# Geronimorz/MCMC-in-Tonga

Hardware: AMD Instinct MI355X
Metric: MCMC proposals/sec (likelihood evals/sec) at 381 rays x N cells (higher is better)
Workload: dtype f64

## Files before the change

### mcmc-in-tonga_amd/csrc/chain_kernels.hip

```cpp
#pragma clang fp contract(off)

#include <hip/hip_runtime.h>

#include <algorithm>
#include <atomic>
#include <climits>
#include <cstddef>
#include <cstdlib>

#include "chain_dev.h"
#include "chain_diag.h"
#include "chain_resident.h"
#include "chain_search.h"
#include "chain_shared.h"
#include "chain_tiles.h"
#include "chain_variant.h"
#include "exact_sum.h"
#include "internal.h"
#include "ray_sum.h"
#include "wave_ops.h"

namespace tdstar {

namespace {
// ... 284 lines not shown
    if constexpr (SMALL && !RLDS) {
        float *a = reinterpret_cast<float *>(lds + L.tlo), *b = reinterpret_cast<float *>(lds + L.thi);
        double *m = reinterpret_cast<double *>(lds + L.tmaxd);
        int *ts = reinterpret_cast<int *>(lds + L.tstart), *tr = reinterpret_cast<int *>(lds + L.tray);
        {
            constexpr int U = 4;
            CopySeg<float, U, NTH> c0{a, d.tile_lo, 3 * NT}, c1{b, d.tile_hi, 3 * NT};
            CopySeg<double, U, NTH> c2{m, d.tile_maxd, NT};
            CopySeg<int, U, NTH> c7{ts, d.tile_start, NT + 1}, c8{tr, d.tile_ray, NT};
            for (int b0 = tid; b0 < 3 * NT; b0 += U * NTH) {
                c0.load(b0); c1.load(b0); c2.load(b0); c7.load(b0); c8.load(b0);
                c0.store(b0); c1.store(b0); c2.store(b0); c7.store(b0); c8.store(b0);
            }
        }
        v.tlo = a; v.thi = b; v.tmaxd = m; v.tstart = ts; v.tray = tr;
        v.thit = reinterpret_cast<int *>(lds + L.thit);
        v.ctm = reinterpret_cast<double *>(lds + L.ctm);
        v.ctm_cap = kCtmLds;
        __syncthreads();
    }
    if constexpr (RLDS) {
        float *a = reinterpret_cast<float *>(lds + L.tlo), *b = reinterpret_cast<float *>(lds + L.thi);
        double *m = reinterpret_cast<double *>(lds + L.tmaxd);
        int *ts = reinterpret_cast<int *>(lds + L.tstart), *ro = reinterpret_cast<int *>(lds + L.rayoff);
        double *p = reinterpret_cast<double *>(lds + L.ptS), *pf = reinterpret_cast<double *>(lds + L.prefix);
        double *t = reinterpret_cast<double *>(lds + L.tS), *sg = reinterpret_cast<double *>(lds + L.sig);
        int *rf = reinterpret_cast<int *>(lds + L.rflag), *od = reinterpret_cast<int *>(lds + L.ord);
        int *tr = reinterpret_cast<int *>(lds + L.tray);
        v.tray = tr;
        {
            constexpr int U = 4;
            CopySeg<float, U, NTH> c0{a, d.tile_lo, 3 * NT}, c1{b, d.tile_hi, 3 * NT};
            CopySeg<double, U, NTH> c2{m, d.tile_maxd, NT}, c3{p, d.ptS, n}, c4{pf, d.prefix, n}, c5{t, d.tS, n},
                c6{sg, d.sig, n};
            CopySeg<int, U, NTH> c7{ts, d.tile_start, NT + 1}, c8{tr, d.tile_ray, NT}, c9{ro, d.ray_off, n + 1},
                c10{od, d.order, d.st->ncells};
            const int most = max(max(3 * NT, NT + 1), max(n + 1, c10.n));
            for (int b0 = tid; b0 < most; b0 += U * NTH) {
                c0.load(b0); c1.load(b0); c2.load(b0); c3.load(b0); c4.load(b0); c5.load(b0);
                c6.load(b0); c7.load(b0); c8.load(b0); c9.load(b0); c10.load(b0);
                c0.store(b0); c1.store(b0); c2.store(b0); c3.store(b0); c4.store(b0); c5.store(b0);
                c6.store(b0); c7.store(b0); c8.store(b0); c9.store(b0); c10.store(b0);
            }
        }
        for (int i = tid; i < n; i += NTH) rf[i] = 0;
        v.tlo = a; v.thi = b; v.tmaxd = m; v.tstart = ts; v.ray_off = ro; v.ptS = p; v.prefix = pf; v.tS = t;
        v.sig = sg; v.rflag = rf; v.ord = od;
        v.cptS = reinterpret_cast<double *>(lds + L.cptS);
        v.cprefix = reinterpret_cast<double *>(lds + L.cprefix);
        v.term = reinterpret_cast<double *>(lds + L.term);
        v.cterm = reinterpret_cast<double *>(lds + L.cterm);
        v.thit = reinterpret_cast<int *>(lds + L.thit);
        v.ctm = reinterpret_cast<double *>(lds + L.ctm);
        v.ctm_cap = NT + 1;
        v.rhit = reinterpret_cast<int *>(lds + L.rhit);
        v.rhit_cap = n;
        __syncthreads();
    }
    const long long t_mirror = prof_on ? clock64() : 0;
    {
        double part = 0.0;
        for (int r = tid; r < n; r += NTH) {
            const double df = v.ptS[r] - v.tS[r];
            const double sg = v.sig[r];
            const double t = ((df * df) * 1.0) / (sg * sg);
            v.term[r] = t;
            part = part + t;
        }
        if constexpr (!RLDS) {
            part = wave_sum_f64(part);
            if (lane == 0) sh.wpart[wv] = part;
        }
    }
    if (tid == 0) {
        const ChainScalars &s0 = *d.st;
        sh.iter = s0.iter;
        sh.evaluations = 0;
        sh.bytes = 0;
        sh.cur = 0;
        sh.defer = 0;
        if (!RLDS) sh.dsum = sh.dabs = 0.0;
        sh.grid_fallbacks32 = 0;
        sh.e_done = sh.b_done = 0;
        geo_fill(sh.geo, d);
        for (int a = 0; a < 5; ++a) sh.proposed[a] = sh.accepted[a] = 0;
        sh.phi = s0.phi;
        sh.ncells = s0.ncells;
        for (int k = 0; k < 3; ++k) sh.lnN[k] = d.logN[max(s0.ncells - 1 + k, 0)];
        sh.nslots = s0.nslots;
        sh.nfree = s0.nfree;
        sh.next_stamp = s0.next_stamp;
        sh.g_op = 0;
        sh.grid_ovf = *d.grid_overflow;
        sh.rT = P.temperature;
        sh.rinv2t = P.inv_2t;
        sh.srv_quit = 0;
        sh.rK = 0;
        for (int k = 0; k < kProfSlots; ++k) sh.prof[k] = 0;
        sh.t_last = clock64();
        sh.dseg.nseg = 0;
    }
    __syncthreads();
    const long long t_init = prof_on ? clock64() : 0;
    unsigned long long *smask = reinterpret_cast<unsigned long long *>(lds + L.smask);
    unsigned long long *cmask = reinterpret_cast<unsigned long long *>(lds + L.cmask);
    const int NS = d.nsuper;
    float *slo = reinterpret_cast<float *>(lds + L.slo), *shi = reinterpret_cast<float *>(lds + L.shi);
    float *smax = reinterpret_cast<float *>(lds + L.smax);
    int *shit = reinterpret_cast<int *>(lds + L.shit);
    const bool super_on = !SMALL && L.super_lds;
    if constexpr (WALK) {
        if constexpr (SMALL) __syncthreads();
        delta_marks(v.term, v.prefix, nullptr, n, smask, wv, delta_words(n), kWv, lane);
        for (int w = tid; w < delta_words(n); w += NTH) cmask[w] = 0ull;
    }
    if constexpr (!SMALL) {
        if (super_on) {
            for (int i = tid; i < 3 * NS; i += NTH) {
                slo[i] = d.super_lo[i];
                shi[i] = d.super_hi[i];
            }
            for (int S = tid; S < NS; S += NTH) {
                double m = 0.0;
                for (int t = S * kTilePts; t < min(NT, (S + 1) * kTilePts); ++t) m = fmax(m, d.tile_maxd[t]);
                smax[S] = f32_up(m);
            }
            if (tid == 0) sh.n_super[0] = sh.n_super[1] = 0;
        }
        __syncthreads();
    }

    if (wv == 0) {
        if (sa.pre) {
            if (lane < iters) draws[lane] = sa.pre[(long long)bchain * sa.pre_stride + lane];
        } else if (!nscript) {
            draws[lane] = tdchain::draw_iteration(d.seed, d.chain, (uint64_t)(sh.iter + lane));
        }
        wave_sync_lds();
        if (mb) {
            if (lane == 0) {
                sh.srv_seq = mb_load(&mb->done);
                sh.srv_quit = 0;
                sh.srv_busy_c = 0;
            }
            wave_sync_lds();
            server_wait(mb, d, v, sh, lane);
        }
        if (rbx) {
            if (lane == 0) sh.rseq = mb_load(&rbx->slot[bchain].done);
            wave_sync_lds();
            round_wait(rbx, bchain, sh, lane, false, sh.phi);
        }
        if (lane == 0 && iters > 0 && !((mb || rbx) && sh.srv_quit)) {
            if (nscript) {
                sh.step_cur = mb ? sh.srv_step[sh.srv_k++] : sa.step[0];
                script_proposal(sh.ps[0], sh.step_cur, sh.nfree, sh.nslots, d.free_slots,
                                [&](int pos) { return v.ord[pos]; });
            }
            else
                make_proposal(sh.ps[0], P, draws[0], sh.ncells, sh.nfree, sh.nslots, d.free_slots, d.cx, d.cy, d.cz,
                              d.czeta, [&](int pos) { return v.ord[pos]; });
            if (sh.ps[0].p.active) sh.proposed[sh.ps[0].p.action] += 1;
            sh.n_tiles = sh.n_changed = sh.n_orphans = sh.n_rays = 0;
            sh.pts_seen = sh.ray_pts = 0;
            sh.k0 = n;
            sh.gs.accept = 0;
// ... 15 lines not shown
            sh.prof[73] += t_init - t_mirror;
            sh.prof[74] += t_now - t_init;
        }
    }
    double phi_r = sh.phi;
    double inv2t_r = sh.rinv2t;
    long long round_end = rbx ? sh.rK : xch ? (long long)rxp->K : LLONG_MAX;
    int cur_r = 0;
    bool pend_r = false;
    bool pend_sup = false;
    int last_action = 0, last_accept = 0;
    long long it_done = 0;
    long long rec_next = LLONG_MAX;
    if constexpr (REC && !ROUNDS)
        if (d.rec.every > 0 && !rbx) rec_next = d.rec.first;
    if constexpr (REC && ROUNDS)
        if (tid == 0) sh.mbox[0] = sh.mbox[1] = -1;
    if (tid == 0) {
        sh.ex_upto = n;
        sh.phi_lo = sh.phi_hi = phi_r;
        if constexpr (!RLDS) {
            double T = 0.0;
            for (int w = 0; w < kWv; ++w) T = T + sh.wpart[w];
            sh.tsum = T;
            sh.terr = kSumSlack * (double)(n + 1) * fabs(T);
        }
    }
    __syncthreads();
    for (long long it = 0; it < iters && !((mb || rbx || xch) && sh.srv_quit); ++it) {
        if (prof_on && tid == 0) sh.t_iter = clock64();
        int sup_n = 0, sup_S = 0, sup_par = 0;
        bool sup_all = false;
        unsigned long long sup_mk = 0ull;
        if constexpr (!SMALL) {
            if (pend_sup) {
                sup_par = (int)((it - 1) & 1);
                const int nsh = sh.n_super[sup_par];
                sup_all = nsh > kListLds;
                sup_n = sup_all ? NS : nsh;
                if ((tid >> 4) < sup_n) {
                    sup_S = sup_all ? (tid >> 4) : shit[sup_par * kListLds + (tid >> 4)];
                    const int t = sup_S * kTilePts + (tid & 15);
                    sup_mk = t < NT ? (unsigned long long)__double_as_longlong(d.tile_maxd[t]) : 0ull;
                }
            }
        }
        if constexpr (WALK) {
            if (pend_r) delta_commit<SMALL ? 1 : 16>(v.prefix, v.cprefix, n, sh.dseg, tid, NTH);
            pend_r = false;
        }
        if constexpr (!SMALL) {
            if (pend_sup) {
                if ((tid >> 4) < sup_n) {
                    const unsigned long long mk = row_max_u64(sup_mk);
                    if ((tid & 15) == 15) smax[sup_S] = f32_up(__longlong_as_double((long long)mk));
                }
                for (int i = (tid >> 4) + NTH / kTilePts; i < sup_n; i += NTH / kTilePts) {
                    const int S = sup_all ? i : shit[sup_par * kListLds + i], t = S * kTilePts + (tid & 15);
                    unsigned long long mk = t < NT ? (unsigned long long)__double_as_longlong(d.tile_maxd[t]) : 0ull;
                    mk = row_max_u64(mk);
                    if ((tid & 15) == 15) smax[S] = f32_up(__longlong_as_double((long long)mk));
                }
                __syncthreads();
                SKEW(1);
                pend_sup = false;
            }
        }
        bool acc_r = false;
        const PState &cur = sh.ps[sh.cur];
        const Proposal p = cur.p;
        const int action = p.action;
        const int ncells = sh.ncells;
        const int slot_k = cur.slot_k;
        const bool eval = cur.eval != 0;
        const double kx = cur.kx, ky = cur.ky, kz = cur.kz;
        const int new_slot = cur.new_slot;
        const double zeta_killed = cur.zeta_killed;
        double czeta = 0.0, zetanew_death = 0.0;
        STAMP(0);
        bool pre_on = false;
        bool nobar = false;
        int pre_q = 0, pre_ray = 0, pre_s = 0;
        double pre_bd = 0.0, pre_x = 0.0, pre_y = 0.0, pre_z = 0.0;
        const bool sroad = !SCRIPT && cur.barren != 0 && p.active && p.valid && P.debug_prior != 1 &&
                           (action == tdchain::kChange || action == tdchain::kDeath);
        if (p.active) {
            const bool kill_q = SCRIPT && mb && action == tdchain::kDeath && sh.step_cur.decision == kDecideLater;
            const bool query = (!nscript && (action == tdchain::kBirth || action == tdchain::kDeath)) || kill_q;
            nobar = kNoBarB && action != tdchain::kBirth && p.valid && P.debug_prior != 1 && !sroad;
            if (eval && !sroad) {
                const bool q0 = action != tdchain::kBirth;
                const bool q1 = action == tdchain::kBirth || action == tdchain::kMove;
                const TileQuery tq0 = tile_query(kx, ky, kz), tq1 = tile_query(p.x, p.y, p.z);
                const int nthr = query ? NTH - 64 : NTH;
                constexpr int TU = SMALL ? 3 : 8;
                if (super_on) {
                    const int par = (int)(it & 1);
                    int *hl = shit + par * kListLds;
                    if (tid < nthr)
                        for (int S0 = tid; S0 < NS; S0 += 4 * nthr) {
                            bool hit[4];
#pragma unroll
                            for (int u = 0; u < 4; ++u) {
                                const int S = min(S0 + u * nthr, NS - 1);
                                const float thr = smax[S] * (1.0f + 0x1p-20f);
                                const bool h0 = tile_may_hit(slo, shi, NS, S, tq0, thr);
                                const bool h1 = tile_may_hit(slo, shi, NS, S, tq1, thr);
                                hit[u] = S0 + u * nthr < NS && ((q0 && h0) || (q1 && h1));
                            }
#pragma unroll
                            for (int u = 0; u < 4; ++u)
                                if (hit[u]) {
                                    const int k = atomicAdd(&sh.n_super[par], 1);
                                    if (k < kListLds) hl[k] = S0 + u * nthr;
                                }
                        }
                    __syncthreads();
                    SKEW(2);
                    const int nsh = sh.n_super[par];
                    const bool all = nsh > kListLds;
                    const int nitems = all ? NS * kTilePts : nsh * kTilePts;
                    if (tid < nthr)
                        for (int i0 = tid; i0 < nitems; i0 += 4 * nthr) {
                            bool hit[4];
                            int4 rec[4];
#pragma unroll
                            for (int u = 0; u < 4; ++u) {
                                const int i = min(i0 + u * nthr, nitems - 1);
                                const int tu = (all ? (i >> 4) : hl[i >> 4]) * kTilePts + (i & 15);
                                const int t = min(tu, NT - 1);
                                const float thr = tile_thr(v.tmaxd[t]);
                                const bool h0 = tile_may_hit(v.tlo, v.thi, NT, t, tq0, thr);
                                const bool h1 = tile_may_hit(v.tlo, v.thi, NT, t, tq1, thr);
                                rec[u] = int4{t, v.tstart[t], v.tray[t], 0};
                                hit[u] = i0 + u * nthr < nitems && tu < NT && ((q0 && h0) || (q1 && h1));
                            }
#pragma unroll
                            for (int u = 0; u < 4; ++u)
                                if (hit[u]) {
                                    const int k = atomicAdd(&sh.n_tiles, 1);
                                    v.thit[k] = rec[u].x;
                                    if (k < v.hrec_cap) v.hrec[k] = rec[u];
                                }
                        }
                } else if (SMALL) {
                    const TileQuery2 tr0 = tile_query2(kx, ky, kz), tr1 = tile_query2(p.x, p.y, p.z);
                    if (tid < nthr) {
                        int npre = 0;
                        int pt[kPre] = {0, 0, 0, 0};
                        for (int b0 = wv * 64; b0 < NT; b0 += TU * nthr) {
                            const int t0 = b0 + lane;
                            bool hit[TU];
                            if constexpr (TD_TILE2) {
                                TileBox bx[TU];
#pragma unroll
                                for (int u = 0; u < TU; ++u)
                                    bx[u] = tile_box(v.tlo, v.thi, v.tmaxd, NT, min(t0 + u * nthr, NT - 1));
                                const int au = __builtin_amdgcn_readfirstlane(action);
                                const bool s0 = au != tdchain::kBirth, s1 = au == tdchain::kBirth || au == tdchain::kMove;
#pragma unroll
                                for (int u = 0; u < TU; ++u) hit[u] = false;
                                if (s0) {
#pragma unroll
                                    for (int u = 0; u < TU; ++u) hit[u] = tile_may_hit2(bx[u], tr0);
                                }
                                if (s1) {
#pragma unroll
                                    for (int u = 0; u < TU; ++u) hit[u] = hit[u] || tile_may_hit2(bx[u], tr1);
// ... 10 lines not shown
                                    hit[u] = t0 + u * nthr < NT && ((q0 && h0) || (q1 && h1));
                                }
                            }
#pragma unroll
                            for (int u = 0; u < TU; ++u) {
                                const unsigned long long m = __ballot(hit[u]);
                                if (m == 0ull) continue;
                                const int first = __builtin_ctzll(m), cnt = __popcll(m);
                                const int rank = __popcll(m & ((1ull << lane) - 1ull));
                                int base = 0;
                                if (lane == first) base = atomicAdd(&sh.n_tiles, cnt);
                                base = __builtin_amdgcn_readlane(base, first);
                                if (hit[u]) {
                                    const int t = t0 + u * nthr, slot = npre + rank;
                                    v.thit[base + rank] = slot < kPre ? (t | INT_MIN) : t;
                                }
                                for (unsigned long long mm = m; mm && npre < kPre; mm &= mm - 1ull) {
                                    const int t = b0 + __builtin_ctzll(mm) + u * nthr;
#pragma unroll
                                    for (int k = 0; k < kPre; ++k) pt[k] = k == npre ? t : pt[k];
                                    ++npre;
                                }
                            }
                        }
                        BPROBE(0);
                        if (npre > 0) {
                            if (lane < kTilePts * npre) {
                                const int g = lane / kTilePts;
                                const int t = g == 0 ? pt[0] : g == 1 ? pt[1] : g == 2 ? pt[2] : pt[3];
                                const int sc = v.tstart[t];
                                if (lane % kTilePts < (sc & 31)) {
                                    const int q = (sc >> 5) + lane % kTilePts;
                                    pre_on = true;
                                    pre_q = q;
                                    pre_ray = v.tray[t];
                                    pre_s = d.best_s[q];
                                    pre_bd = d.best_d[q];
                                    pre_x = d.px[q];
                                    pre_y = d.py[q];
                                    pre_z = d.pz[q];
                                }
                            }
                        }
                    }
                } else if (tid < nthr)
                    for (int t0 = tid; t0 < NT; t0 += TU * nthr) {
                        bool hit[TU];
#pragma unroll
                        for (int u = 0; u < TU; ++u) {
                            const int t = min(t0 + u * nthr, NT - 1);
                            const float thr = tile_thr(v.tmaxd[t]);
                            const bool h0 = tile_may_hit(v.tlo, v.thi, NT, t, tq0, thr);
                            const bool h1 = tile_may_hit(v.tlo, v.thi, NT, t, tq1, thr);
                            hit[u] = t0 + u * nthr < NT && ((q0 && h0) || (q1 && h1));
                        }
#pragma unroll
                        for (int u = 0; u < TU; ++u)
                            if (hit[u]) {
                                const int k = atomicAdd(&sh.n_tiles, 1), t = t0 + u * nthr;
                                v.thit[k] = t;
                                if (!SMALL && k < v.hrec_cap) v.hrec[k] = int4{t, v.tstart[t], v.tray[t], 0};
                            }
                    }
            }
            BPROBE(1);
            if (nobar && !(query && wv == kWv - 1)) {
                __builtin_amdgcn_fence(__ATOMIC_RELEASE, "workgroup");
                if (lane == 0) atomicAdd(&sh.b_done, 1);
                SKEW(3);
            }
            if (RLDS && action == tdchain::kDeath && nscript) {
                const int sthr = query ? NTH - 64 : NTH;
                if constexpr (RLDS) {
                    if (tid < sthr)
                        for (int j = (int)p.index + 1 + tid; j < ncells; j += sthr) d.order_tmp[j] = v.ord[j];
                }
            }
            if (query && wv == kWv - 1) {
                const bool birth = action == tdchain::kBirth;
                if (nobar && lane == 0) atomicAdd(&sh.b_done, 1);
                const Nearest r = wave_nearest(d, v, sh, lane, birth ? p.x : kx, birth ? p.y : ky, birth ? p.z : kz,
                                               birth ? -1 : slot_k, -1, 0.0, 0.0, 0.0, 0.0);
                if (lane == 0) sh.q_zeta = r.z;
            }
        }
        if (!nobar && !(sroad && action == tdchain::kChange)) {
            __syncthreads();
            SKEW(4);
            if (p.active && action == tdchain::kBirth) czeta = sh.q_zeta;
            if (p.active && action == tdchain::kDeath) zetanew_death = sh.q_zeta;
        }
        BPROBE(2);
        Proposal pp = p;
        if (p.active && action == tdchain::kBirth && !nscript) tdchain::birth_zeta(P, pp, czeta);
        STAMP(1);
        const bool can_spec = !nscript && it + 1 < iters && ((it + 1) & 63) != 0;
        if (pp.active && pp.valid) {
            const bool fwd = P.debug_prior != 1;
            int no = 0;
            if (fwd && !sroad) {
                if (!nscript && tid == NTH - 64)
                    sh.ap = tdchain::alpha_parts(P, pp, czeta, zeta_killed,
                                                 nobar && action == tdchain::kDeath ? sh.q_zeta : zetanew_death,
                                                 sh.lnN);

                const int nt = sh.n_tiles;
                const double zeta_k = slot_k >= 0 ? zeta_killed : 0.0;
                int seen = 0;
                auto point = [&](int q, int ray, int s, double bd, double qx, double qy, double qz) {
                    if (action == tdchain::kBirth) {
                        const double dd = dist2(pp.x, pp.y, pp.z, qx, qy, qz);
                        if (dd < bd) mark(d, v, sh, q, ray, new_slot, dd, pp.zeta, s);
                    } else if (action == tdchain::kChange) {
                        if (s == slot_k) mark(d, v, sh, q, ray, s, bd, pp.zeta, s);
                    } else if (s == slot_k) {
                        const int o = atomicAdd(&sh.n_orphans, 1);
                        d.orphans[o] = q;
                        if (o < kOrphanLds) sh.orph[o] = OrphanRec{qx, qy, qz, q, ray};
                    } else if (action == tdchain::kMove) {
                        const double dd = dist2(pp.x, pp.y, pp.z, qx, qy, qz);
                        if (dd < bd || (dd == bd && s >= 0 && d.stamp[slot_k] < d.stamp[s]))
                            mark(d, v, sh, q, ray, slot_k, dd, zeta_k, s);
                    }
                };
                if constexpr (SMALL) {
                    if (pre_on) {
                        ++seen;
                        point(pre_q, pre_ray, pre_s, pre_bd, pre_x, pre_y, pre_z);
                    }
                    if (nobar)
                        SPIN_WAIT(__hip_atomic_load(&sh.b_done, __ATOMIC_ACQUIRE, __HIP_MEMORY_SCOPE_WORKGROUP) < kWv, 1);
                    const int nt = sh.n_tiles;
                    for (int item = tid; item < nt * kTilePts; item += NTH) {
                        const int t = v.thit[item / kTilePts];
                        if (t < 0) continue;
                        const int sc = v.tstart[t];
                        if (item % kTilePts >= (sc & 31)) continue;
                        const int q = (sc >> 5) + item % kTilePts;
                        ++seen;
                        const int s = d.best_s[q];
                        const double bd = d.best_d[q];
                        const double qx = d.px[q], qy = d.py[q], qz = d.pz[q];
                        point(q, v.tray[t], s, bd, qx, qy, qz);
                    }
                } else {
                    constexpr int CU = 4;
                    for (int item0 = tid; item0 < nt * kTilePts; item0 += CU * NTH) {
                        int qq[CU], rr[CU], ss[CU];
                        double bb[CU], xx[CU], yy[CU], zz[CU];
#pragma unroll
                        for (int u = 0; u < CU; ++u) {
                            const int item = item0 + u * NTH;
                            const int4 rec = v.tile_rec(min(item, nt * kTilePts - 1) / kTilePts);
                            const int sc = rec.y;
                            const bool in = item < nt * kTilePts && item % kTilePts < (sc & 31);
                            const int q = in ? (sc >> 5) + item % kTilePts : 0;
                            qq[u] = in ? q : -1;
                            rr[u] = rec.z;
                            ss[u] = d.best_s[q];
                            bb[u] = d.best_d[q];
                            xx[u] = d.px[q];
                            yy[u] = d.py[q];
                            zz[u] = d.pz[q];
                        }
#pragma unroll
                        for (int u = 0; u < CU; ++u)
                            if (qq[u] >= 0) {
                                ++seen;
                                point(qq[u], rr[u], ss[u], bb[u], xx[u], yy[u], zz[u]);
// ... 314 lines not shown
                    const double wsum = wave_sum_f64((p0 + p1) + (p2 + p3));
                    if (lane == 0) sh.wpart[wv] = wsum;
                    __syncthreads();
                    SKEW(13);
                }
            }
            if (RLDS && !nscript && action == tdchain::kDeath && lane == 0) {
                if (wv != 0) {
                    int a, b;
                    shift_range((int)p.index, ncells, wv, kWv - 1, a, b);
                    if (b > a) sh.shift_edge[wv] = v.ord[b - 1];
                } else {
                    sh.shift_done = 0;
                }
            }
            if (wv == 0) {
                const int k0 = sh.k0;
                if (fwd) {
                    if (!WALK || !nscript) {
                        bool exact = nscript != 0;
                        if (k0 >= n) phi_n = phi_r;
                        if (!exact && k0 < n) {
                            double Sa = Tp, Ea = Ep;
                            if (anchor) {
                                Sa = 0.0;
                                if constexpr (WALK) {
                                    for (int w = 0; w < kWv; ++w) Sa = Sa + sh.wpart[w];
                                } else {
                                    double part = 0.0;
                                    for (int k = lane; k < n; k += 64) part = part + v.term[k];
                                    Sa = wave_sum_f64(part);
                                }
                                Ea = kSumSlack * (double)(n + 1) * fabs(Sa);
                            }
                            if (!RLDS && lane == 0) {
                                sh.b_T = Sa;
                                sh.b_E = Ea;
                            }
                            const double b_lo = (Sa - Ea) * (1.0 - 1e-9), b_hi = (Sa + Ea) * (1.0 + 1e-9);
                            const int sure = tdchain::decide_sure(sh.ap, pp.log_u, (sh.phi_lo - b_hi) * inv2t_r,
                                                                  (sh.phi_hi - b_lo) * inv2t_r);
                            if (sure != 0) {
                                bdec = sure > 0 ? 2 : 1;
                            } else {
                                const bool lo = lane == 0;
                                const int a = lane < 2 ? (int)tdchain::accept_t(P, inv2t_r, pp, lo ? sh.phi_lo : sh.phi_hi,
                                                                               lo ? b_hi : b_lo, czeta, zeta_killed,
                                                                               zetanew_death, sh.lnN)
                                                       : 0;
                                const int a_min = __builtin_amdgcn_readlane(a, 0), a_max = __builtin_amdgcn_readlane(a, 1);
                                bdec = a_min != a_max ? 0 : a_min ? 2 : 1;
                            }
                            if ((rbx || xch) && it + 1 == round_end) bdec = 0;
                            if constexpr (REC)
                                if (it + 1 == rec_next) bdec = 0;
                            if (d.exact_every > 0 && (it % d.exact_every) == d.exact_every - 1) bdec = 0;
                            exact = bdec == 0;
                            phi_n = Sa;
                            if (bdec == 2 && lane == 0) {
                                sh.ex_upto = min(sh.ex_upto, k0);
                                sh.b_lo = b_lo;
                                sh.b_hi = b_hi;
                            }
                        }
                        if (exact && k0 < n) {
                            const ExactPhis ex = exact_sums(v.term, v.prefix, v.cprefix, v.cterm, v.rflag, sh, n, lane,
                                                            true, k0, phi_r, phi_n);
                            phi_r = ex.phi;
                            phi_n = ex.phi_n;
                            if (prof_on && lane == 0) sh.prof[65] += 1;
                        }
                        if (prof_on && lane == 0 && k0 < n) sh.prof[64] += n - k0;
                    } else {
                        double C = k0 > 0 ? v.prefix[k0 - 1] : 0.0;
                        if (k0 < n) {
                            C = delta_walk(v.term, v.prefix, v.rflag, k0, n, C, smask, cmask, v.cprefix, sh.dseg, lane,
                                           prof_on ? &sh.prof[72] : nullptr);
                            if (prof_on && lane == 0) sh.prof[64] += n - k0;
                        }
                        phi_n = k0 < n ? C : sh.phi;
                    }
                }
                if (prof_on && lane == 0) sh.prof[66] += clock64() - tF;
            }
            if (tid == 0) {
                const bool acc = nscript ? sh.step_cur.decision == 1
                                 : bdec != 0 ? bdec == 2
                                             : tdchain::accept_t(P, inv2t_r, pp, phi_r, phi_n, czeta, zeta_killed,
                                                                 zetanew_death, sh.lnN);
                acc_r = acc;
                sh.gs = Shared::GSnap{sh.n_changed, sh.n_rays, sh.n_tiles, sh.k0, acc ? 1 : 0};
                sh.defer = bdec == 2 ? 1 : 0;
                sh.phi_n = phi_n;
                if (prof_on) sh.prof[67] += clock64() - tF;
                if (acc || (mb && sh.step_cur.decision == kDecideLater)) {
                    sh.g_op = action == tdchain::kBirth ? 2 : action == tdchain::kDeath ? 1
                              : action == tdchain::kMove ? 3 : 4;
                    sh.g_slot = action == tdchain::kBirth ? new_slot : slot_k;
                    sh.g_ox = kx;
                    sh.g_oy = ky;
                    sh.g_oz = kz;
                    sh.g_nx = pp.x;
                    sh.g_ny = pp.y;
                    sh.g_nz = pp.z;
                    sh.g_nzeta = pp.zeta;
                    if (acc) atomicAdd((unsigned long long *)&sh.accepted[action], 1ull);
                }
                if (prof_on && bdec == 1) atomicAdd((unsigned long long *)&sh.prof[14], 1ull);
            } else if (spec_in_F && tid == 64) {
                if (can_spec) {
                    make_proposal<true>(sh.ps[sh.cur ^ 1], P, draws[(it + 1) & 63], ncells, sh.nfree, sh.nslots,
                                        d.free_slots, d.cx, d.cy, d.cz, d.czeta, [&](int pos) { return v.ord[pos]; }, d.own);
                    sh.spec_ok = 1;
                }
            } else if (wv == kWv - 1 || (kWv >= 6 && wv == kWv - 2)) {
                if (wv == kWv - 1)
                    grid_prefetch(d, sh, lane, action, action == tdchain::kBirth ? new_slot : slot_k, kx, ky,
                                  kz, pp.x, pp.y, pp.z);
                if (wv == (kWv >= 6 ? kWv - 2 : kWv - 1)) {
                    if (prof_on && lane == 0) {
                        if (sroad) sh.prof[action == tdchain::kDeath ? 35 : 45] += 1;
                        sh.prof[68] += sh.n_tiles;
                        sh.prof[69] += sh.pts_seen;
                        sh.prof[70] += sh.n_changed;
                        sh.prof[71] += sh.n_rays;
                    }
                    if (lane == 0 && fwd) {
                        atomicAdd((unsigned long long *)&sh.evaluations, 1ull);
                        const bool owns_none = !SCRIPT && ((action == tdchain::kChange && sh.n_changed == 0) ||
                                                          (action == tdchain::kDeath && no == 0));
                        atomicAdd((unsigned long long *)&sh.bytes,
                                  (unsigned long long)((owns_none  ? 0ll
                                                        : super_on ? (long long)NS * 32 +
                                                                         (long long)sh.n_super[it & 1] * kTilePts * 32 +
                                                                         (long long)sh.pts_seen * 36
                                                                   : (long long)NT * 32 + (long long)sh.pts_seen * 36) +
                                                       (long long)(no + (action <= 2 ? 1 : 0)) * 27 * 8 * 32 +
                                                       (RLDS ? 0ll : (long long)sh.ray_pts * 17) + (long long)(n - sh.k0) * 28));
                    }
                    if (lane == 0 && (action == tdchain::kBirth || action == tdchain::kDeath)) {
                        sh.lnN_far[0] = d.logN[max(ncells - 2, 0)];
                        sh.lnN_far[1] = d.logN[ncells + 2];
                    }
                }
            } else if (wv >= 2 && wv <= (kWv >= 6 ? kWv - 3 : 2) && fwd && action != tdchain::kChange) {
                const int nt = sh.n_tiles;
                constexpr int MU = 4, MS = (kWv >= 6 ? kWv - 4 : 1) * 64;
                if constexpr (RLDS) {
                    for (int i = tid - 128; i < nt * kTilePts; i += MS) {
                        const int sc = v.tile_rec(i / kTilePts).y;
                        const int q = (sc >> 5) + (i % kTilePts);
                        unsigned long long mk = 0ull;
                        if (i % kTilePts < (sc & 31)) {
                            const double cd = d.cand_d[q], bd = d.best_d[q];
                            mk = (unsigned long long)__double_as_longlong(d.cand_flag[q] ? cd : bd);
                        }
                        mk = row_max_u64(mk);
                        if ((i % kTilePts) == kTilePts - 1) v.ctm_put(i / kTilePts, __longlong_as_double((long long)mk));
                    }
                } else
                for (int i0 = tid - 128; i0 < nt * kTilePts; i0 += MU * MS) {
                    int q[MU];
                    bool in[MU];
#pragma unroll
                    for (int u = 0; u < MU; ++u) {
                        const int i = min(i0 + u * MS, nt * kTilePts - 1);
                        const int sc = v.tile_rec(i / kTilePts).y;
                        in[u] = i0 + u * MS < nt * kTilePts && (i % kTilePts) < (sc & 31);
                        q[u] = in[u] ? (sc >> 5) + (i % kTilePts) : 0;
                    }
                    double cd[MU], bd[MU];
                    unsigned char cf[MU];
#pragma unroll
                    for (int u = 0; u < MU; ++u) {
                        cd[u] = d.cand_d[q[u]];
                        bd[u] = d.best_d[q[u]];
                        cf[u] = d.cand_flag[q[u]];
                    }
#pragma unroll
                    for (int u = 0; u < MU; ++u) {
                        const int i = i0 + u * MS;
                        if (i >= nt * kTilePts) break;
                        unsigned long long mk = 0ull;
                        if (in[u]) mk = (unsigned long long)__double_as_longlong(cf[u] ? cd[u] : bd[u]);
                        mk = row_max_u64(mk);
                        if ((i % kTilePts) == kTilePts - 1) v.ctm_put(i / kTilePts, __longlong_as_double((long long)mk));
                    }
                }
            }
            if (prof_on && lane == 0)
                atomicAdd((unsigned long long *)&sh.prof[56 + wv], (unsigned long long)(clock64() - tF));
            __syncthreads();
            STAMP(5);
            SKEW(14);
            const int nc = sh.gs.nc, nr = sh.gs.nr;
            if (nscript && sdec != 1 && !early && wv == 0) server_report(sa.out, v, sh, n, lane, sh.phi_n);
            if (mb && sdec == kDecideLater) {
                if (wv == 0) server_wait(mb, d, v, sh, lane);
                __syncthreads();
                SKEW(15);
                if (tid == 0) acc_r = sh.gs.accept != 0;
            }
            constexpr int kW = NTH - 64;
            const int w = tid - 64;
// ... 166 lines not shown
                }
            }
            if ((rbx || xch) && it + 1 == round_end) {
                {
                    phi_r = exact_sums(v.term, v.prefix, v.cprefix, v.cterm, v.rflag, sh, n, lane, false, n, phi_r, 0.0).phi;
                    if (lane == 0) sh.phi = phi_r;
                }
                if constexpr (REC && ROUNDS) {
                    long long ri = -1;
                    if (rbx) {
                        if (lane == 0) ri = mb_load(&rbx->slot[bchain].rec_i);
                    } else if (d.rec.every > 0) {
                        const RoundX &x = *rxp;
                        const int lv = lane < x.R ? x.lev[bchain * x.R + lane] : -1;
                        const int mine = __shfl(lv, (x.rank * x.local + bchain) & 63);
                        const long long jr = (it + 1) / x.K;
                        if (mine == 0 && jr >= d.rec.first && (jr - d.rec.first) % d.rec.every == 0)
                            ri = (jr - d.rec.first) / d.rec.every;
                    }
                    if (lane == 0) {
                        sh.mbox[0] = d.rec.every > 0 ? ri : -1;
                        sh.mbox[1] = it + 1;
                    }
                }
                if (rbx) {
                    round_wait(rbx, bchain, sh, lane, true, phi_r);
                    round_end = it + 1 + sh.rK;
                } else {
                    const long long Kx = rxp->K;
                    round_exchange(*rxp, bchain, (it + 1) / Kx - 1, sh, lane, phi_r);
                    round_end = it + 1 + Kx;
                }
                inv2t_r = sh.rinv2t;
            }
            if (it + 1 < iters && !((mb || rbx || xch) && sh.srv_quit)) {
                if (((it + 1) & 63) == 0 && !nscript) {
                    wave_sync_lds();
                    if (sa.pre) {
                        if (it + 1 + lane < iters) draws[lane] = sa.pre[(long long)bchain * sa.pre_stride + it + 1 + lane];
                    } else {
                        draws[lane] = tdchain::draw_iteration(d.seed, d.chain, (uint64_t)(iter0 + it + 1 + lane));
                    }
                    wave_sync_lds();
                }
                if (lane == 0) {
                    const bool acc = acc_r;
                    const PState &g = sh.ps[cur_r ^ 1];
                    const bool keep = sh.spec_ok && can_spec &&
                                      (!acc || ((action == tdchain::kChange || action == tdchain::kMove) &&
                                                g.slot_k != slot_k));
                    if (keep) {
                        cur_r ^= 1;
                        sh.cur = cur_r;
                        if (prof_on && g.barren) sh.prof[55] += 1;
                        if (acc && action != tdchain::kChange && sh.gs.nc != 0) {
                            if (prof_on && g.barren) sh.prof[25] += 1;
                            sh.ps[cur_r].barren = 0;
                        }
                    } else {
                        const bool killed = RLDS && acc && action == tdchain::kDeath;
                        if (killed && !nscript)
                            SPIN_WAIT(__hip_atomic_load(&sh.shift_done, __ATOMIC_ACQUIRE, __HIP_MEMORY_SCOPE_WORKGROUP) <
                                          kWv - 1,
                                      1000000);
                        auto slot_at = [&](int pos) {
                            return (killed && nscript && pos >= (int)pp.index) ? d.order_tmp[pos + 1] : v.ord[pos];
                        };
                        if (nscript) {
                            sh.step_cur = mb ? sh.srv_step[sh.srv_k++] : sa.step[it + 1];
                            script_proposal(sh.ps[cur_r], sh.step_cur, sh.nfree, sh.nslots, d.free_slots, slot_at);
                        }
                        else
                            make_proposal(sh.ps[cur_r], P, draws[(it + 1) & 63], sh.ncells, sh.nfree, sh.nslots,
                                          d.free_slots, d.cx, d.cy, d.cz, d.czeta, slot_at);
                    }
                    const tdchain::Proposal &np = sh.ps[cur_r].p;
                    if (np.active) atomicAdd((unsigned long long *)&sh.proposed[np.action], 1ull);
                    sh.spec_ok = 0;
                    sh.n_tiles = sh.n_changed = sh.n_orphans = sh.n_rays = 0;
                    if (!RLDS) sh.dsum = sh.dabs = 0.0;
                    sh.n_super[(it + 1) & 1] = 0;
                    sh.pts_seen = sh.ray_pts = 0;
                    sh.e_done = sh.b_done = 0;
                    sh.k0 = n;
                }
            }
        }
        STAMP(13);
        it_done = it + 1;
        __syncthreads();
        STAMP(6);
        SKEW(17);
        if constexpr (REC && ROUNDS) {
            if (sh.mbox[1] == it + 1 && sh.mbox[0] >= 0) {
                record_round_sample(d, v.ord, v.ptS, sh, sh.mbox[0], iter0 + it, last_action, last_accept, tid, NTH);
                __syncthreads();
                SKEW(20);
            }
        }
        if constexpr (REC && !ROUNDS) {
            if (it + 1 == rec_next) {
                record_sample(d, v.ord, v.ptS, sh, it, iter0, last_action, last_accept, tid, NTH);
                rec_next += d.rec.every;
                __syncthreads();
                SKEW(19);
            }
        }
    }

    const long long t_loop_end = prof_on ? clock64() : 0;
    {
        if (wv == 0) {
            phi_r = exact_sums(v.term, v.prefix, v.cprefix, v.cterm, v.rflag, sh, n, lane, false, n, phi_r, 0.0).phi;
            if (lane == 0) sh.phi = phi_r;
        }
        __syncthreads();
    }
    if constexpr (WALK) {
        if (pend_r) delta_commit<SMALL ? 1 : 16>(v.prefix, v.cprefix, n, sh.dseg, tid, NTH);
        if constexpr (SMALL) __syncthreads();
    }
    if constexpr (SMALL) {
        for (int i = tid; i < NT; i += NTH) d.tile_maxd[i] = v.tmaxd[i];
        if constexpr (RLDS) {
            for (int i = tid; i < n; i += NTH) {
                d.ptS[i] = v.ptS[i];
                d.prefix[i] = v.prefix[i];
            }
            for (int i = tid; i < sh.ncells; i += NTH) d.order[i] = v.ord[i];
        }
    }
    if (tid == 0) {
        ChainScalars &s = *d.st;
        s.iter = iter0 + it_done;
        s.evaluations += sh.evaluations;
        s.bytes += sh.bytes;
        for (int a = 0; a < 5; ++a) {
            s.proposed[a] += sh.proposed[a];
            s.accepted[a] += sh.accepted[a];
        }
        s.phi = sh.phi;
        s.ncells = sh.ncells;
        s.nslots = sh.nslots;
        s.nfree = sh.nfree;
        s.next_stamp = sh.next_stamp;
        if (iters > 0) {
            s.last_action = last_action;
            s.last_accept = last_accept;
        }
        if (prof_on) {
            sh.prof[77] += clock64() - t_loop_end;
            sh.prof[78] += 1;
        }
        for (int k = 0; k < kProfSlots; ++k) s.prof[k] += sh.prof[k];
        s.prof[15] += sh.grid_fallbacks32;
        if (d.st_host) *d.st_host = s;
        if (mb) {
            __threadfence_system();
            mb_store(&mb->exited, 1);
        }
        if (rbx) {
            __threadfence_system();
            mb_store(&rbx->slot[bchain].exited, 1);
        }
    }
}
// ... 159 lines not shown
```

### mcmc-in-tonga_amd/csrc/chain_shared.h

```cpp
#pragma once
#include <hip/hip_runtime.h>

#include <algorithm>
#include <cstddef>

#include "chain_dev.h"
#include "exact_sum.h"
#include "internal.h"

namespace tdstar {

namespace {

using tdchain::Proposal;

constexpr int kWaves = kChainThreads / 64;
static_assert(kTilePts == 16, "a tile is one 16-lane DPP row (row_max_u64)");
constexpr int kOrphanLds = 96;
constexpr int kPre = 64 / kTilePts;
static_assert(kPre == 4, "the preload slots are four registers");
constexpr int kCtmLds = 256;
constexpr int kListLds = 1024;
constexpr int kBatchOrphans = 64;
constexpr int kBatchCand = 192;
// ... 39 lines not shown
    const int *count;
    const CellEntry *buckets;
    const int *bslot;
    int gx, gy, gz, sealed;
};
__device__ __forceinline__ void geo_fill(GridGeo &g, const DevChain &d) {
    const CellGrid &G = d.grid;
    g.x0 = G.x0; g.y0 = G.y0; g.z0 = G.z0;
    g.ix = G.ix; g.iy = G.iy; g.iz = G.iz;
    g.hx = G.hx; g.hy = G.hy; g.hz = G.hz;
    g.ex = G.ex; g.ey = G.ey; g.ez = G.ez;
    for (int a = 0; a < 3; ++a) {
        g.lo[a] = G.lo[a];
        g.hi[a] = G.hi[a];
    }
    g.count = d.bucket_count;
    g.buckets = d.buckets;
    g.bslot = d.bslot;
    g.gx = G.gx; g.gy = G.gy; g.gz = G.gz;
    g.sealed = G.sealed;
    const double h3[3] = {G.hx, G.hy, G.hz}, e3[3] = {G.ex, G.ey, G.ez};
    const int g3[3] = {G.gx, G.gy, G.gz};
    double lb0 = __builtin_huge_val();
    for (int a = 0; a < 3; ++a) {
        if (g3[a] < 3) continue;
        const double gap = (h3[a] - 2.0 * e3[a]) * (1.0 - 0x1p-30);
        const double f = gap > 0.0 ? gap * gap : 0.0;
        lb0 = f < lb0 ? f : lb0;
    }
    g.lb0 = grid_lb_close(lb0);
}

struct Shared {
    GridGeo geo;
    PState ps[2];
    int cur, spec_ok;
    int defer;
    double phi_n;
    int ex_upto;
    double phi_lo, phi_hi, b_lo, b_hi;
    int n_tiles, n_changed, n_orphans, n_rays, k0;
    struct GSnap {
        int nc, nr, nt, k0, accept;
    } gs;
    int ob_lo[3], ob_hi[3], ob_ncand, ob_nfb;
    int n_super[2];
    int pts_seen, ray_pts;
    int e_done;
    int b_done;
    int g_op, g_slot;
    int gp_bo, gp_co, gp_pos, gp_bn, gp_cn;
    CellEntry gp_last;
    int gp_last_slot;
    double g_nzeta;
    double g_ox, g_oy, g_oz, g_nx, g_ny, g_nz;
    long long iter, evaluations, bytes;
    long long proposed[5], accepted[5];
    double phi;
    int ncells, nslots, nfree;
    long long next_stamp;
    double lnN[3];
    double lnN_far[2];
    double q_zeta;
    int grid_fallbacks32;
    int grid_ovf;
    ScriptStep step_cur;
    ScriptStep srv_step[kMaxScript];
    int srv_n, srv_k, srv_quit;
    double rT, rinv2t;
    long long rseq;
    int rK, rskip;
    long long srv_seq, srv_busy_c, srv_busy_w;
    long long mbox[40];
    OrphanRec orph[kOrphanLds];
    ChgRec chg[kChgLds];
    tdchain::AlphaParts ap;
    DeltaSegs dseg;
    long long prof[kProfSlots], t_last, t_iter;
    double tsum, terr, dsum, dabs, b_T, b_E;
    double wpart[kChainThreads / 64];
    int shift_done;
    int shift_edge[kChainThreads / 64];
    int dbg_site[kChainThreads / 64];
};

struct LdsPlan {
    size_t scratch, draws, smask, cmask, slo, shi, smax, shit, hrec, rhitl, tlo, thi, tmaxd, tstart, thit, ctm, tray, rayoff, ptS, prefix, cptS, cprefix, term, cterm,
        tS, sig, rflag, rhit, ord, total;
    bool super_lds;
    bool lists_lds;
};

constexpr size_t kLdsBudget = 160 * 1024;
constexpr size_t kDrawsBudget = (size_t)256 << 20;

__host__ __device__ inline size_t align16(size_t x) { return (x + 15) & ~(size_t)15; }

__host__ __device__ inline LdsPlan lds_plan(int ntiles, int n, int cap, bool small, int waves = kWaves,
                                            bool rays_lds = true) {
    LdsPlan L{};
    size_t o = align16(sizeof(Shared));
    L.scratch = o; o += align16(sizeof(double) * waves * (small ? 96 : 192));
    L.draws = o; o += align16(sizeof(tdchain::Draws) * 64);
    if (!small || kSmallWalk) {
        L.smask = o; o += align16(sizeof(unsigned long long) * delta_words(n));
        L.cmask = o; o += align16(sizeof(unsigned long long) * delta_words(n));
    }
    if (small) {
        L.tlo = o; o += align16(sizeof(float) * 3 * ntiles);
        L.thi = o; o += align16(sizeof(float) * 3 * ntiles);
        L.tmaxd = o; o += align16(sizeof(double) * ntiles);
        L.tstart = o; o += align16(sizeof(int) * (ntiles + 1));
        L.thit = o; o += align16(sizeof(int) * (ntiles + 1));
        L.ctm = o; o += align16(sizeof(double) * (rays_lds ? ntiles + 1 : kCtmLds));
        L.tray = o; o += align16(sizeof(int) * ntiles);
        if (rays_lds) {
            L.rayoff = o; o += align16(sizeof(int) * (n + 1));
            L.ptS = o; o += align16(sizeof(double) * n);
            L.prefix = o; o += align16(sizeof(double) * n);
            L.cptS = o; o += align16(sizeof(double) * n);
            L.cprefix = o; o += align16(sizeof(double) * n);
            L.term = o; o += align16(sizeof(double) * n);
            L.cterm = o; o += align16(sizeof(double) * n);
            L.tS = o; o += align16(sizeof(double) * n);
            L.sig = o; o += align16(sizeof(double) * n);
            L.rflag = o; o += align16(sizeof(int) * n);
            L.rhit = o; o += align16(sizeof(int) * n);
            L.ord = o; o += align16(sizeof(int) * cap);
        }
    } else {
        size_t q = o;
        L.hrec = q; q += align16(sizeof(int4) * kListLds);
        L.rhitl = q; q += align16(sizeof(int) * kListLds);
        L.lists_lds = q <= kLdsBudget;
        if (L.lists_lds) o = q;
        const int ns = (ntiles + kTilePts - 1) / kTilePts;
        q = o;
        L.slo = q; q += align16(sizeof(float) * 3 * ns);
        L.shi = q; q += align16(sizeof(float) * 3 * ns);
        L.smax = q; q += align16(sizeof(float) * ns);
        L.shit = q; q += align16(sizeof(int) * 2 * kListLds);
        L.super_lds = q <= kLdsBudget;
        if (L.super_lds) o = q;
    }
    L.total = o;
    return L;
}

inline ChainLaunchFacts launch_facts(const DevChain *host, int nchains) {
    ChainLaunchFacts f{};
    f.packed = f.tiles_ok = f.all_auto = true;
    for (int b = 0; b < nchains; ++b) {
        const DevChain &d = host[b];
        f.small = std::max(f.small, lds_plan(d.ntiles, d.n, d.cap, true).total);
        f.big = std::max(f.big, lds_plan(d.ntiles, d.n, d.cap, false).total);
        f.half = std::max(f.half, lds_plan(d.ntiles, d.n, d.cap, false, kWaves / 2).total);
        f.hyb = std::max(f.hyb, lds_plan(d.ntiles, d.n, d.cap, true, kWaves / 2, false).total);
        f.force_hbm = f.force_hbm || d.lds_mode >= 1;
        f.packed = f.packed && d.lds_mode >= 2;
        f.tiles_ok = f.tiles_ok && d.lds_mode == 2;
        f.all_auto = f.all_auto && d.lds_mode == 0;
        f.rec = f.rec || d.rec.every > 0;
    }
    f.nchains = nchains;
    f.budget = kLdsBudget;
    return f;
// ... 59 lines not shown
```

### profiles/chain_phases.py

```python
#!/usr/bin/env python3
import ctypes
import json
import os
import sys
import time

import numpy as np

ROOT = os.path.dirname(os.path.dirname(os.path.abspath(__file__)))
sys.path.insert(0, ROOT)
import tonga

PHASES = ["(loop top)", "B tiles + birth/death query", "C points", "D orphans", "E ray sums",
          "F chi2 + accept || next proposal, tile maxima", "G commit + grid update + next proposal"]


def main():
    N = int(sys.argv[1]) if len(sys.argv) > 1 else 5000
    iters = int(sys.argv[2]) if len(sys.argv) > 2 else 20000
    nrays = int(sys.argv[3]) if len(sys.argv) > 3 else 0
    tt = tonga.load()
    ds = tt.synthetic_rays(nrays, seed=5) if nrays > 0 else tt.load_data_Tonga()
    ctx = tt.TdContext.from_datastruct(ds)
    prm = tt.define_TDstructrure().replace(max_cells=2 * N)
    ch = tt.Chain(ctx, tt.chain_params(prm, ds, seed=1000, chain=1), tt.random_model(N, 3))
    ch.run(2000 if nrays == 0 else 200)
    L = tt.lib()
    out0 = (ctypes.c_int64 * 80)()
    L.tdt_chain_profile(ch.h, 1, out0)
    st0 = ch.stats()
    t0 = time.perf_counter()
    ch.run(iters)
    el = time.perf_counter() - t0
    out = (ctypes.c_int64 * 80)()
    L.tdt_chain_profile(ch.h, 0, out)
    cyc = np.array(out[:7], dtype=np.float64) - np.array(out0[:7], dtype=np.float64)
    cyc[6] += (out[12] - out0[12]) + (out[13] - out0[13])
    fallbacks = int(out[15] - out0[15])
    tot = cyc.sum()
    st1 = ch.stats()
    prop = np.array(st1["proposed"], dtype=np.float64) - np.array(st0["proposed"], dtype=np.float64)
    act = np.array(out[8:12], dtype=np.float64) - np.array(out0[8:12], dtype=np.float64)
    per_action = {a: round(c / max(k, 1), 1) for a, c, k in zip(["birth", "death", "change", "move"], act, prop)}
    res = {"cells": N, "iters": iters, "us_per_iter_wall": el / iters * 1e6,
           "cycles_per_iter": tot / iters, "grid_fallbacks": fallbacks,
           "phases": {p: {"share": round(c / tot, 4), "cycles_per_iter": round(c / iters, 1)}
                      for p, c in zip(PHASES, cyc)},
           "cycles_per_proposal_by_action": per_action,
           "early_rejections": int(out[14] - out0[14]),
           "rejections": int(sum(prop) - (sum(ch.stats()["accepted"]) - sum(st0["accepted"]))),
           "G sub-phases per iter (tid 0)": {
               "commit": round((out[12] - out0[12]) / iters, 1),
               "next proposal": round((out[13] - out0[13]) / iters, 1),
               "final barrier": round((out[6] - out0[6]) / iters, 1)}}
    names = PHASES[:6] + ["G commit", "G next proposal", "final barrier"]
    res["phases_by_action (cycles per proposal)"] = {
        a: {names[j]: round((out[16 + 10 * i + j] - out0[16 + 10 * i + j]) / max(prop[i], 1), 1) for j in range(9)}
        for i, a in enumerate(["birth", "death", "change", "move"])}
    res["F per wave (cycles per iter): chi2 scan, next proposal, tile maxima x4, bound, grid prefetch"] = [
        round((out[56 + w] - out0[56 + w]) / iters, 1) for w in range(8)]
    ev = max(sum(prop), 1)
    res["chi2 tail terms per proposal"] = round((out[64] - out0[64]) / ev, 1)
    res["chi2 scan rounds per proposal"] = round((out[65] - out0[65]) / ev, 2)
    res["per evaluated proposal: tiles hit, points seen, points changed, rays changed"] = [
        round((out[k] - out0[k]) / ev, 1) for k in (68, 69, 70, 71)]
    short = [int(out[k] - out0[k]) for k in (35, 45)]
    res["short road (the cell owns no ray point): deaths, changes, share of all proposals"] = short + [
        round(sum(short) / ev, 4)]
    res["guesses adopted with a barren cell, of those with the flag cleared at adoption"] = [
        int(out[k] - out0[k]) for k in (55, 25)]
    res["chi2 walk (rays in HBM) per proposal: events, batch-load cycles, walk cycles, terms one by one"] = [
        round((out[k] - out0[k]) / ev, 1) for k in (72, 73, 74, 75)]
    res["F wave 0: cycles to scan end / to decision (per iter)"] = [round((out[k] - out0[k]) / iters, 1)
                                                                     for k in (66, 67)]
    print(json.dumps(res, indent=1))


if __name__ == "__main__":
    main()
```

Baseline: 166,800.

## Detect barren cells from live ownership count and drop death-query barrier

For change and death proposals, the kernel now also reads the cell's owned-point count from global memory at the top of the loop, so cells that own no ray point take the short road even when the cached barren flag is clear. For short-road deaths, the nearest-cell query wave signals completion through an LDS counter instead of a workgroup barrier, and wave 0 spin-waits on that counter only right before the acceptance decision. Grid prefetch moves to another wave in that case. This adds an atomic global load per proposal and spin-wait logic, plus profiling counters that pack two values into one slot.

```diff
diff --git a/mcmc-in-tonga_amd/csrc/chain_kernels.hip b/mcmc-in-tonga_amd/csrc/chain_kernels.hip
--- a/mcmc-in-tonga_amd/csrc/chain_kernels.hip
+++ b/mcmc-in-tonga_amd/csrc/chain_kernels.hip
@@ -390,6 +390,7 @@
         if (!RLDS) sh.dsum = sh.dabs = 0.0;
         sh.grid_fallbacks32 = 0;
         sh.e_done = sh.b_done = 0;
+        if constexpr (kNoBarB) sh.q_done = 0;
         geo_fill(sh.geo, d);
         for (int a = 0; a < 5; ++a) sh.proposed[a] = sh.accepted[a] = 0;
         sh.phi = s0.phi;
@@ -571,8 +572,19 @@
         bool nobar = false;
         int pre_q = 0, pre_ray = 0, pre_s = 0;
         double pre_bd = 0.0, pre_x = 0.0, pre_y = 0.0, pre_z = 0.0;
-        const bool sroad = !SCRIPT && cur.barren != 0 && p.active && p.valid && P.debug_prior != 1 &&
-                           (action == tdchain::kChange || action == tdchain::kDeath);
+        bool sroad = false;
+        int own_top = -1;
+        if constexpr (!SCRIPT) {
+            if ((action == tdchain::kChange || action == tdchain::kDeath) && p.active && p.valid) {
+                const bool up = cur.barren != 0;
+                if (!up)
+                    own_top = __builtin_amdgcn_readfirstlane(
+                        __hip_atomic_load((const __attribute__((address_space(1))) int *)(d.own + slot_k),
+                                          __ATOMIC_RELAXED, __HIP_MEMORY_SCOPE_AGENT));
+                sroad = (up || own_top == 0) && P.debug_prior != 1;
+            }
+        }
+        const bool qroad = kNoBarB && sroad && action == tdchain::kDeath;
         if (p.active) {
             const bool kill_q = SCRIPT && mb && action == tdchain::kDeath && sh.step_cur.decision == kDecideLater;
             const bool query = (!nscript && (action == tdchain::kBirth || action == tdchain::kDeath)) || kill_q;
@@ -749,9 +761,14 @@
                 const Nearest r = wave_nearest(d, v, sh, lane, birth ? p.x : kx, birth ? p.y : ky, birth ? p.z : kz,
                                                birth ? -1 : slot_k, -1, 0.0, 0.0, 0.0, 0.0);
                 if (lane == 0) sh.q_zeta = r.z;
-            }
-        }
-        if (!nobar && !(sroad && action == tdchain::kChange)) {
+                if (qroad) {
+                    __builtin_amdgcn_fence(__ATOMIC_RELEASE, "workgroup");
+                    if (lane == 0) atomicAdd(&sh.q_done, 1);
+                    SKEW(22);
+                }
+            }
+        }
+        if (!nobar && !(sroad && action == tdchain::kChange) && !qroad) {
             __syncthreads();
             SKEW(4);
             if (p.active && action == tdchain::kBirth) czeta = sh.q_zeta;
@@ -1232,6 +1249,11 @@
                     }
                 }
                 if (prof_on && lane == 0) sh.prof[66] += clock64() - tF;
+                if (qroad) {
+                    SPIN_WAIT(__hip_atomic_load(&sh.q_done, __ATOMIC_ACQUIRE, __HIP_MEMORY_SCOPE_WORKGROUP) < 1,
+                              1000000000);
+                    zetanew_death = sh.q_zeta;
+                }
             }
             if (tid == 0) {
                 const bool acc = nscript ? sh.step_cur.decision == 1
@@ -1263,13 +1285,18 @@
                                         d.free_slots, d.cx, d.cy, d.cz, d.czeta, [&](int pos) { return v.ord[pos]; }, d.own);
                     sh.spec_ok = 1;
                 }
-            } else if (wv == kWv - 1 || (kWv >= 6 && wv == kWv - 2)) {
-                if (wv == kWv - 1)
+            } else if (wv == kWv - 1 || (kWv >= 6 && wv == kWv - 2) || (qroad && wv == kWv - 3)) {
+                if (wv == (qroad ? kWv - 3 : kWv - 1))
                     grid_prefetch(d, sh, lane, action, action == tdchain::kBirth ? new_slot : slot_k, kx, ky,
                                   kz, pp.x, pp.y, pp.z);
                 if (wv == (kWv >= 6 ? kWv - 2 : kWv - 1)) {
                     if (prof_on && lane == 0) {
                         if (sroad) sh.prof[action == tdchain::kDeath ? 35 : 45] += 1;
+                        if (own_top >= 0 && fwd)
+                            sh.prof[action == tdchain::kDeath ? 7 : 75] += own_top == 0 ? 1ll : 1ll << 32;
+                        if (!SCRIPT && fwd && !sroad &&
+                            ((action == tdchain::kChange && sh.n_changed == 0) || (action == tdchain::kDeath && no == 0)))
+                            sh.prof[action == tdchain::kDeath ? 35 : 45] += 1ll << 32;
                         sh.prof[68] += sh.n_tiles;
                         sh.prof[69] += sh.pts_seen;
                         sh.prof[70] += sh.n_changed;
@@ -1602,6 +1629,7 @@
                     sh.n_super[(it + 1) & 1] = 0;
                     sh.pts_seen = sh.ray_pts = 0;
                     sh.e_done = sh.b_done = 0;
+                    if constexpr (kNoBarB) sh.q_done = 0;
                     sh.k0 = n;
                 }
             }
diff --git a/mcmc-in-tonga_amd/csrc/chain_shared.h b/mcmc-in-tonga_amd/csrc/chain_shared.h
--- a/mcmc-in-tonga_amd/csrc/chain_shared.h
+++ b/mcmc-in-tonga_amd/csrc/chain_shared.h
@@ -145,6 +145,7 @@
     int shift_done;
     int shift_edge[kChainThreads / 64];
     int dbg_site[kChainThreads / 64];
+    int q_done;
 };
 
 struct LdsPlan {
diff --git a/profiles/chain_phases.py b/profiles/chain_phases.py
--- a/profiles/chain_phases.py
+++ b/profiles/chain_phases.py
@@ -64,13 +64,19 @@
     res["chi2 scan rounds per proposal"] = round((out[65] - out0[65]) / ev, 2)
     res["per evaluated proposal: tiles hit, points seen, points changed, rays changed"] = [
         round((out[k] - out0[k]) / ev, 1) for k in (68, 69, 70, 71)]
-    short = [int(out[k] - out0[k]) for k in (35, 45)]
+    lo, hi = (lambda k: int(out[k] - out0[k]) & 0xffffffff), (lambda k: int(out[k] - out0[k]) >> 32)
+    short = [lo(k) for k in (35, 45)]
     res["short road (the cell owns no ray point): deaths, changes, share of all proposals"] = short + [
         round(sum(short) / ev, 4)]
+    res["point counts read at the loop top: deaths owning none / some, changes owning none / some"] = [
+        lo(7), hi(7), lo(75), hi(75)]
+    barren_full = [hi(k) for k in (35, 45)]
+    res["on the full path though the cell owned no point: deaths, changes, share of all proposals"] = barren_full + [
+        round(sum(barren_full) / ev, 4)]
     res["guesses adopted with a barren cell, of those with the flag cleared at adoption"] = [
         int(out[k] - out0[k]) for k in (55, 25)]
-    res["chi2 walk (rays in HBM) per proposal: events, batch-load cycles, walk cycles, terms one by one"] = [
-        round((out[k] - out0[k]) / ev, 1) for k in (72, 73, 74, 75)]
+    res["chi2 walk (rays in HBM) per proposal: events, batch-load cycles, walk cycles"] = [
+        round((out[k] - out0[k]) / ev, 1) for k in (72, 73, 74)]
     res["F wave 0: cycles to scan end / to decision (per iter)"] = [round((out[k] - out0[k]) / iters, 1)
                                                                      for k in (66, 67)]
     print(json.dumps(res, indent=1))
```

Result: faster. 169,300 (median of 6 runs) (+1.5%).
